# vlongle/pixie

Hardware: AMD Instinct MI355X
Metric: voxels/s (128^3 U-Net fwd) + MPM particle-steps/s (higher is better)
Workload: dtype f32 (operands split fp16 hi+lo, 3 f16 MFMAs/product, fp32 accumulate); 1 GPU; 128^3x64 feature grid -> SegmentationUNet+RegressionUNet forward (+argmax/one-hot combine), 1 scene per GPU per step; grid=128, feature_channels=64, parallelism=scene-parallel x1, executor=c+hip_graph

## Files before the change

include/pixie_hip.h:

```cpp
#ifndef PIXIE_HIP_H
#define PIXIE_HIP_H

#include <stdint.h>

#ifdef __cplusplus
extern "C" {
#endif

const char* pixie_last_error(void);
const char* pixie_build_arch(void);

typedef struct pixie_mpm pixie_mpm;

int pixie_mpm_create(pixie_mpm** out, int n_particles, int n_grid, double grid_lim);
int pixie_mpm_destroy(pixie_mpm* h);
int pixie_mpm_regrid(pixie_mpm* h, int n_grid, double grid_lim, void* stream);

int pixie_mpm_set_field(pixie_mpm* h, const char* name, const void* d_src, int64_t count, void* stream);
int pixie_mpm_get_field(pixie_mpm* h, const char* name, void* d_dst, int64_t count, void* stream);
int pixie_mpm_fill_field(pixie_mpm* h, const char* name, double value, void* stream);

int pixie_mpm_set_scalar(pixie_mpm* h, const char* key, double value);
int pixie_mpm_get_scalar(pixie_mpm* h, const char* key, double* value);

// ... 72 lines not shown
    int32_t in_d, in_h, in_w;
    int32_t upsample;
    int32_t stride;
    int32_t ksize;
    const float* d_pro_a; const float* d_pro_b;
    const float* d_gamma; const float* d_beta;
    int32_t act;
    const float* d_w; const float* d_bias;
    int32_t c_out;
    const float* d_residual;
    float* d_out;
    const void* d_w16;
    const uint32_t* d_in_amax0; const uint32_t* d_in_amax1;
    float in_bound;
    float* d_out_stats;
    uint32_t* d_out_amax;
    void* d_workspace;
    int32_t out_d, out_h, out_w;
    const float* d_skip_in0; int32_t skip_c0;
    const float* d_skip_in1; int32_t skip_c1;
    const void* d_skip_w16; const float* d_skip_bias;
    const uint32_t* d_skip_amax0; const uint32_t* d_skip_amax1;
    int32_t w16_subpixel;
} pixie_conv_desc;

int pixie_conv_cout_padded(int c_out);
int pixie_conv_pack_weights(const float* d_w_oidhw, float* d_w_packed, int c_out, int c_in, int ksize, void* stream);
int64_t pixie_conv_packed16_bytes(int c_out, int c_in, int ksize);
int pixie_conv_pack_weights_f16x2(const float* d_w_oidhw, void* d_packed, int c_out, int c_in, int ksize, void* stream);
int64_t pixie_conv_subpixel_bytes(int c_out, int c_in);
int pixie_conv_pack_weights_subpixel(const float* d_w_oidhw, void* d_packed, int c_out, int c_in, void* stream);
int pixie_conv3d_forward(const pixie_conv_desc* desc, void* stream);
int64_t pixie_conv_stats_floats(const pixie_conv_desc* desc);
int64_t pixie_conv_workspace_bytes(const pixie_conv_desc* desc);
int pixie_stats_finalize(const float* d_stats, const pixie_conv_desc* desc, double* d_sums, void* stream);
int pixie_stats_norm_finalize(const float* d_stats0, const pixie_conv_desc* desc0, double* d_sums0, const float* d_stats1,
                              const pixie_conv_desc* desc1, double* d_sums1, int c1, int64_t spatial, int mode, int groups,
                              double eps, const float* d_weight, const float* d_bias, float* d_a, float* d_b, void* stream);
int pixie_conv_skip_foldable(const pixie_conv_desc* desc);

int pixie_channel_sums(const float* d_x, int channels, int64_t spatial, double* d_sums, void* stream);
int pixie_channel_stats(const float* d_x, int channels, int64_t spatial, double* d_sums, uint32_t* d_amax, void* stream);
int pixie_tensor_amax(const float* d_x, int64_t count, uint32_t* d_slot, void* stream);
int pixie_norm_finalize(const double* d_sums, int channels, int64_t spatial, int mode, int groups, double eps,
                        const float* d_weight, const float* d_bias, float* d_a, float* d_b, void* stream);

// ... 168 lines not shown
```

pixie_amd/_lib.py:

```python
from __future__ import annotations

import ctypes as C
import os

_HERE = os.path.dirname(os.path.abspath(__file__))
LIB_PATH = os.path.join(_HERE, "libpixie_hip.so")
DIAG_LIB_PATH = os.path.join(_HERE, "libpixie_hip_diag.so")


class PixieHipError(RuntimeError):
    pass


class BCDesc(C.Structure):
    _fields_ = [("type", C.c_int32), ("surface_type", C.c_int32), ("reset", C.c_int32), ("pad_", C.c_int32),
                ("point", C.c_double * 3), ("size", C.c_double * 3), ("velocity", C.c_double * 3),
                ("normal", C.c_double * 3), ("start_time", C.c_double), ("end_time", C.c_double),
                ("friction", C.c_double)]


class PModDesc(C.Structure):
    _fields_ = [("type", C.c_int32), ("pad_", C.c_int32),
                ("point", C.c_double * 3), ("size", C.c_double * 3), ("force", C.c_double * 3),
                ("velocity", C.c_double * 3), ("normal", C.c_double * 3), ("h1", C.c_double * 3),
# ... 2 lines not shown
                ("start_time", C.c_double), ("end_time", C.c_double)]


class ConvDesc(C.Structure):
    _fields_ = [("d_in0", C.c_void_p), ("c0", C.c_int32),
                ("d_in1", C.c_void_p), ("c1", C.c_int32),
                ("in_d", C.c_int32), ("in_h", C.c_int32), ("in_w", C.c_int32),
                ("upsample", C.c_int32), ("stride", C.c_int32), ("ksize", C.c_int32),
                ("d_pro_a", C.c_void_p), ("d_pro_b", C.c_void_p),
                ("d_gamma", C.c_void_p), ("d_beta", C.c_void_p),
                ("act", C.c_int32),
                ("d_w", C.c_void_p), ("d_bias", C.c_void_p),
                ("c_out", C.c_int32),
                ("d_residual", C.c_void_p), ("d_out", C.c_void_p),
                ("d_w16", C.c_void_p), ("d_in_amax0", C.c_void_p), ("d_in_amax1", C.c_void_p),
                ("in_bound", C.c_float),
                ("d_out_stats", C.c_void_p), ("d_out_amax", C.c_void_p),
                ("d_workspace", C.c_void_p),
                ("out_d", C.c_int32), ("out_h", C.c_int32), ("out_w", C.c_int32),
                ("d_skip_in0", C.c_void_p), ("skip_c0", C.c_int32),
                ("d_skip_in1", C.c_void_p), ("skip_c1", C.c_int32),
                ("d_skip_w16", C.c_void_p), ("d_skip_bias", C.c_void_p),
                ("d_skip_amax0", C.c_void_p), ("d_skip_amax1", C.c_void_p),
                ("w16_subpixel", C.c_int32)]


class UNetConfigC(C.Structure):
    _fields_ = [("feature_channels", C.c_int32), ("cond_dim", C.c_int32), ("model_channels", C.c_int32), ("num_res_blocks", C.c_int32),
                ("n_channel_mult", C.c_int32), ("channel_mult", C.c_int32 * 8),
                ("n_attention_resolutions", C.c_int32), ("attention_resolutions", C.c_int32 * 8),
                ("grid_size", C.c_int32), ("out_channels", C.c_int32), ("precision", C.c_int32)]


class BatchSched(C.Structure):
    _fields_ = [("dt", C.c_double), ("steps_per_chunk", C.c_int32), ("n_chunks", C.c_int32), ("n_out", C.c_int32), ("pad_", C.c_int32),
                ("shift", C.c_double * 3), ("scale", C.c_double), ("mean", C.c_double * 3), ("inv_rotation", C.c_double * 9),
                ("d_pos", C.c_void_p), ("d_cov", C.c_void_p)]


class BatchSplatOut(C.Structure):
    _fields_ = [("d_log_scale", C.c_void_p), ("d_quat", C.c_void_p)]


class FieldDesc(C.Structure):
    _fields_ = [("d_pred", C.c_void_p), ("d_mask", C.c_void_p),
                ("d_axis_x", C.c_void_p), ("d_axis_y", C.c_void_p), ("d_axis_z", C.c_void_p),
                ("n_classes", C.c_int32), ("d", C.c_int32), ("h", C.c_int32), ("w", C.c_int32),
# ... 170 lines not shown
```

pixie_amd/csrc/conv3d_f16x3.hip:

```cpp
#include <hip/hip_runtime.h>

#include <cstdlib>
#include <map>
#include <string>
#include <type_traits>

#include "../../include/pixie_hip.h"
#include "common.h"
#include "conv_plan.h"

namespace pixie {

typedef float f32x16 __attribute__((ext_vector_type(16)));
typedef _Float16 f16x8 __attribute__((ext_vector_type(8)));

constexpr int kW16HeaderU4 = 4;

struct Conv16Args {
    const float* in0; const float* in1;
    int c0, cin;
    int ID, IH, IW;
    int LD, LH, LW;
    int ups;
    int stride;
// ... 583 lines not shown

__device__ inline void block_channel_sums(const StatParts& P, int c, double* r, double& o1, double& o2) {
    double s1 = 0.0, s2 = 0.0;
    for (int t = threadIdx.x; t < P.n; t += 256) {
        const size_t k = ((size_t)c * P.cstride + (size_t)t * P.tstride) * 2;
        if (P.f64) { const double2 v = *reinterpret_cast<const double2*>(static_cast<const double*>(P.p) + k); s1 += v.x; s2 += v.y; }
        else { const float2 v = *reinterpret_cast<const float2*>(static_cast<const float*>(P.p) + k); s1 += v.x; s2 += v.y; }
    }
    for (int off = 32; off > 0; off >>= 1) { s1 += __shfl_down(s1, off, 64); s2 += __shfl_down(s2, off, 64); }
    if ((threadIdx.x & 63) == 0) { r[2 * (threadIdx.x >> 6)] = s1; r[2 * (threadIdx.x >> 6) + 1] = s2; }
    __syncthreads();
    o1 = r[0] + r[2] + r[4] + r[6]; o2 = r[1] + r[3] + r[5] + r[7];
    __syncthreads();
}

__global__ __launch_bounds__(256) void stats_finalize_kernel(StatParts P, double* __restrict__ sums) {
    const int c = blockIdx.x;
    __shared__ double r[8];
    double s1, s2;
    block_channel_sums(P, c, r, s1, s2);
    if (threadIdx.x == 0) { sums[2 * c] = s1; sums[2 * c + 1] = s2; }
}

__global__ __launch_bounds__(256) void stats_norm_finalize_kernel(StatParts P0, double* sums0, int c0, StatParts P1, double* sums1, int channels,
                                                                  double spatial, int mode, int groups, double eps,
                                                                  const float* __restrict__ weight, const float* __restrict__ bias,
                                                                  float* __restrict__ a, float* __restrict__ b) {
    __shared__ double r[8];
    const int cpg = mode == 0 ? 1 : channels / groups;
    const int first = blockIdx.x * cpg;
    double s1 = 0.0, s2 = 0.0;
    for (int k = first; k < first + cpg; ++k) {
        const bool in0 = k < c0;
        const StatParts& P = in0 ? P0 : P1;
        double* sums = in0 ? sums0 : sums1;
        const int kc = in0 ? k : k - c0;
        double t1, t2;
        if (P.n > 0) {
            block_channel_sums(P, kc, r, t1, t2);
            if (threadIdx.x == 0) { sums[2 * kc] = t1; sums[2 * kc + 1] = t2; }
        } else {
            t1 = sums[2 * kc]; t2 = sums[2 * kc + 1];
        }
        s1 += t1; s2 += t2;
    }
    const double cnt = mode == 0 ? spatial : spatial * cpg;
    const double mean = s1 / cnt;
    double var = s2 / cnt - mean * mean;
    if (var < 0.0) var = 0.0;
    const double rstd = 1.0 / sqrt(var + eps);
    for (int k = first + threadIdx.x; k < first + cpg; k += 256) {
        if (mode == 0) {
            a[k] = (float)rstd;
            b[k] = (float)(-mean * rstd);
        } else {
            const double w = weight ? (double)weight[k] : 1.0;
            const double bb = bias ? (double)bias[k] : 0.0;
            a[k] = (float)(rstd * w);
            b[k] = (float)(bb - mean * rstd * w);
        }
    }
}

__global__ __launch_bounds__(256) void splitk_reduce_kernel(const float* __restrict__ partial, int slices, long n_elems, long osp,
                                                            const float* __restrict__ bias, const float* residual, float* out) {
    const long i = (long)blockIdx.x * 256 + threadIdx.x;
    if (i >= n_elems) return;
    float v = partial[i];
    for (int s = 1; s < slices; ++s) v += partial[(size_t)s * n_elems + i];
    if (bias) v += bias[i / osp];
    if (residual) v += residual[i];
    out[i] = v;
}

constexpr int kReduceSeg = 4096;
template <bool VEC>
__global__ __launch_bounds__(256) void splitk_reduce_stats_kernel(const float* __restrict__ partial, int slices, long n_elems, long osp,
                                                                  const float* __restrict__ bias, const float* residual, float* out,
                                                                  double* __restrict__ stats, unsigned* out_amax) {
    const int c = blockIdx.y;
    const long seg0 = (long)blockIdx.x * kReduceSeg;
    const size_t base = (size_t)c * osp;
    const float bv = bias ? bias[c] : 0.0f;
    double s1 = 0.0, s2 = 0.0;
    float mx = 0.0f;
    if (VEC) {
#pragma unroll
        for (int k = 0; k < kReduceSeg / 1024; ++k) {
            const long j = seg0 + k * 1024 + (long)threadIdx.x * 4;
            if (j < osp) {
                const size_t i = base + j;
                float4 v = *reinterpret_cast<const float4*>(partial + i);
                for (int s = 1; s < slices; ++s) {
                    const float4 q = *reinterpret_cast<const float4*>(partial + (size_t)s * n_elems + i);
                    v.x += q.x; v.y += q.y; v.z += q.z; v.w += q.w;
                }
                if (bias) { v.x += bv; v.y += bv; v.z += bv; v.w += bv; }
                if (residual) {
                    const float4 q = *reinterpret_cast<const float4*>(residual + i);
                    v.x += q.x; v.y += q.y; v.z += q.z; v.w += q.w;
                }
                *reinterpret_cast<float4*>(out + i) = v;
// ... 11 lines not shown
                const size_t i = base + j;
                float v = partial[i];
                for (int s = 1; s < slices; ++s) v += partial[(size_t)s * n_elems + i];
                if (bias) v += bv;
                if (residual) v += residual[i];
                out[i] = v;
                const double x = v;
                s1 += x; s2 += x * x; mx = fmaxf(mx, fabsf(v));
            }
        }
    }
    for (int off = 32; off > 0; off >>= 1) {
        s1 += __shfl_down(s1, off, 64);
        s2 += __shfl_down(s2, off, 64);
        mx = fmaxf(mx, __shfl_down(mx, off, 64));
    }
    __shared__ double r[8];
    __shared__ float rmx[4];
    const int lane = threadIdx.x & 63, wave = threadIdx.x >> 6;
    if (lane == 0) { r[2 * wave] = s1; r[2 * wave + 1] = s2; rmx[wave] = mx; }
    __syncthreads();
    if (threadIdx.x == 0) {
        double* dst = stats + ((size_t)c * gridDim.x + blockIdx.x) * 2;
        dst[0] = r[0] + r[2] + r[4] + r[6];
        dst[1] = r[1] + r[3] + r[5] + r[7];
        const unsigned m = __float_as_uint(fmaxf(fmaxf(rmx[0], rmx[1]), fmaxf(rmx[2], rmx[3])));
        if (out_amax && m > __hip_atomic_load(out_amax, __ATOMIC_RELAXED, __HIP_MEMORY_SCOPE_AGENT)) atomicMax(out_amax, m);
    }
}

__global__ __launch_bounds__(256) void amax_kernel(const float* __restrict__ x, long n, unsigned* __restrict__ slot) {
    float m = 0.0f;
    const long stride = (long)gridDim.x * 256 * 4;
    long i = ((long)blockIdx.x * 256 + threadIdx.x) * 4;
    if ((reinterpret_cast<size_t>(x) & 15) == 0) {
        for (; i + 3 < n; i += stride) {
            const float4 v = *reinterpret_cast<const float4*>(x + i);
            m = fmaxf(fmaxf(m, fabsf(v.x)), fmaxf(fabsf(v.y), fmaxf(fabsf(v.z), fabsf(v.w))));
        }
        for (long k = i; k < n && k < i + 4; ++k) m = fmaxf(m, fabsf(x[k]));
    } else {
        for (long k = (long)blockIdx.x * 256 + threadIdx.x; k < n; k += (long)gridDim.x * 256) m = fmaxf(m, fabsf(x[k]));
    }
    for (int off = 32; off > 0; off >>= 1) m = fmaxf(m, __shfl_down(m, off, 64));
    if ((threadIdx.x & 63) == 0 && m > 0.0f) atomicMax(slot, __float_as_uint(m));
}

__global__ void pack_weights_f16x2_kernel(const float* __restrict__ src, uint4* __restrict__ dst, int cout, int cin, int taps,
                                          int coutp, const unsigned* __restrict__ amax_bits) {
    const int KG = cin >> 3;
// ... 221 lines not shown
int conv3d_f16x3_forward(const pixie_conv_desc* d, const ConvPlan& p, hipStream_t st) {
    PX_REQUIRE(p.refusal != CONV_BAD_STRIDE, "f16x3 conv: stride must be 1, or 2 for a 3^3 kernel");
    PX_REQUIRE(p.refusal != CONV_BAD_CHANNELS, "f16x3 conv: c_in must be a multiple of 16 (got %d+%d)", d->c0, d->c1);
    PX_REQUIRE(d->d_in_amax0 != nullptr || d->in_bound > 0.0f, "f16x3 conv: needs d_in_amax0 or a positive in_bound");
    PX_REQUIRE(d->c1 == 0 || d->d_in_amax0 == nullptr || d->d_in_amax1 != nullptr, "f16x3 conv: second input needs its own amax slot");
    PX_REQUIRE(p.refusal != CONV_BAD_SUBPIXEL, "f16x3 conv: sub-pixel weights need upsample = 1, ksize = 3, stride = 1 and no folded skip");
    Conv16Args a = conv16_args(d, p);
    a.w16 = reinterpret_cast<const uint4*>(d->d_w16);
    a.amax0 = d->d_in_amax0; a.amax1 = (d->c1 > 0) ? d->d_in_amax1 : nullptr; a.in_bound = d->in_bound;
    a.stats = d->d_out_stats; a.out_amax = d->d_out_amax;
    if (d->d_skip_w16) {
        PX_REQUIRE(p.skip_foldable, "f16x3 conv: this launch cannot fold a skip convolution (pixie_conv_skip_foldable)");
        PX_REQUIRE(d->d_skip_in0 && d->d_skip_amax0 && (d->skip_c1 == 0 || (d->d_skip_in1 && d->d_skip_amax1)), "f16x3 conv: folded skip needs its inputs and their amax slots");
        a.sk_in0 = d->d_skip_in0; a.sk_in1 = d->d_skip_in1; a.sk_c0 = d->skip_c0; a.sk_cin = d->skip_c0 + d->skip_c1;
        a.sk_w16 = reinterpret_cast<const uint4*>(d->d_skip_w16); a.sk_bias = d->d_skip_bias;
        a.sk_amax0 = d->d_skip_amax0; a.sk_amax1 = d->skip_c1 > 0 ? d->d_skip_amax1 : nullptr;
    }
    if (p.slices > 1) {
        a.partial = static_cast<float*>(d->d_workspace);
        a.stats = nullptr; a.out_amax = nullptr;
    }
    PX_REQUIRE(p.refusal != CONV_BAD_LDS, "f16x3 conv: tile needs %zu B of LDS", p.lds_bytes);
    PX_REQUIRE(p.f16x3(), "f16x3 conv: bad sizes");
    if (int rc = launch(conv16_kernel(p), p, a, st)) return rc;
    if (p.slices == 1) return 0;
    const long osp = (long)a.OD * a.OH * a.OW, n_elems = (long)a.cout * osp;
    if (d->d_out_stats) {
        const dim3 rgrid((unsigned)reduce_segments(osp), (unsigned)a.cout);
        double* rstats = reinterpret_cast<double*>(d->d_out_stats);
        PX_REQUIRE((reinterpret_cast<size_t>(rstats) & 7) == 0, "f16x3 conv: d_out_stats of a split-K launch must be 8-byte aligned");
        const bool vec = osp % 4 == 0 && ((reinterpret_cast<size_t>(a.partial) | reinterpret_cast<size_t>(a.residual) | reinterpret_cast<size_t>(a.out)) & 15) == 0;
        if (vec) hipLaunchKernelGGL(splitk_reduce_stats_kernel<true>, rgrid, dim3(256), 0, st, a.partial, p.slices, n_elems, osp, a.bias, a.residual,
                                    a.out, rstats, d->d_out_amax);
        else hipLaunchKernelGGL(splitk_reduce_stats_kernel<false>, rgrid, dim3(256), 0, st, a.partial, p.slices, n_elems, osp, a.bias, a.residual,
                                a.out, rstats, d->d_out_amax);
    } else {
        hipLaunchKernelGGL(splitk_reduce_kernel, dim3((unsigned)((n_elems + 255) / 256)), dim3(256), 0, st, a.partial, p.slices, n_elems, osp,
                           a.bias, a.residual, a.out);
    }
    PX_CHECK_HIP(hipGetLastError());
    return 0;
}

int conv3d_exact_forward(const pixie_conv_desc* d, const ConvPlan& p, hipStream_t st) {
    PX_REQUIRE(p.refusal != CONV_BAD_LDS, "exact conv: tile needs %zu B of LDS", p.lds_bytes);
    PX_REQUIRE(p.path == CONV_EXACT_TILED, "exact conv: bad sizes");
    Conv16Args a = conv16_args(d, p);
    a.wf = d->d_w;
    a.in_bound = 1.0f;
    return launch(conv16_kernel(p), p, a, st);
}

}

using namespace pixie;

static ConvPlan plan_of(const pixie_conv_desc* d) { return d ? conv_plan(conv_shape_of(d)) : ConvPlan{}; }
static StatParts stat_parts(const ConvPlan& p, const void* stats) { return StatParts{stats, p.stats.n, p.stats.cstride, p.stats.tstride, p.stats.f64}; }
// ... 116 lines not shown
```

pixie_amd/csrc/conv3d_mfma.hip:

```cpp
#include <hip/hip_runtime.h>

#include "../../include/pixie_hip.h"
#include "common.h"
#include "conv_plan.h"

namespace pixie {

typedef float f32x16 __attribute__((ext_vector_type(16)));

struct ConvArgs {
    const float* in0; const float* in1;
    int c0, cin;
    int ID, IH, IW;
    int LD, LH, LW;
    int ups;
    int stride;
    int OD, OH, OW;
    const float* pro_a; const float* pro_b; const float* gamma; const float* beta;
    int act;
    const float* w; const float* bias;
    int cout, coutp;
    const float* residual; float* out;
    int TX, TY, TZ, lTX, lTY;
    int tiles_x, tiles_y, tiles_z;
// ... 177 lines not shown
    const int taps = ksize * ksize * ksize;
    const int coutp = pixie_conv_cout_padded(c_out);
    const long total = (long)taps * c_in * coutp;
    hipLaunchKernelGGL(pack_weights_kernel, dim3(cdiv(total, 256)), dim3(256), 0, as_stream(stream), d_w, d_packed, c_out, c_in, taps, coutp);
    PX_CHECK_HIP(hipGetLastError());
    return 0;
}

extern "C" int pixie_conv3d_forward(const pixie_conv_desc* d, void* stream) {
    PX_REQUIRE(d && d->d_in0 && (d->d_w || d->d_w16) && d->d_out, "pixie_conv3d_forward: null pointer in descriptor");
    PX_REQUIRE(d->ksize == 1 || d->ksize == 3, "pixie_conv3d_forward: ksize must be 1 or 3 (got %d)", d->ksize);
    PX_REQUIRE(d->stride == 1 || d->stride == 2, "pixie_conv3d_forward: stride must be 1 or 2 (got %d)", d->stride);
    PX_REQUIRE(d->upsample == 0 || d->upsample == 1, "pixie_conv3d_forward: upsample must be 0 or 1");
    PX_REQUIRE(d->c0 > 0 && d->c1 >= 0 && (d->c1 == 0 || d->d_in1), "pixie_conv3d_forward: bad channel split");
    PX_REQUIRE(d->c_out > 0 && d->in_d > 0 && d->in_h > 0 && d->in_w > 0, "pixie_conv3d_forward: bad sizes");
    PX_REQUIRE((d->d_pro_a == nullptr) == (d->d_pro_b == nullptr), "pixie_conv3d_forward: pro_a/pro_b must come together");
    PX_REQUIRE((d->d_gamma == nullptr) == (d->d_beta == nullptr), "pixie_conv3d_forward: gamma/beta must come together");
    PX_REQUIRE(!(d->d_gamma && d->upsample) || (d->d_w16 && d->w16_subpixel),
               "pixie_conv3d_forward: spatial affine with upsample needs the sub-pixel path (w16_subpixel), with gamma/beta of the stored grid");

    const ConvPlan p = conv_plan(conv_shape_of(d));
    if (d->d_w16) return conv3d_f16x3_forward(d, p, as_stream(stream));
    PX_REQUIRE(!d->d_skip_w16, "pixie_conv3d_forward: a folded skip convolution needs the f16x3 path (d_w16)");
    if (p.path != CONV_FIRST_GEN) return conv3d_exact_forward(d, p, as_stream(stream));

    ConvArgs a{};
    a.in0 = d->d_in0; a.in1 = d->d_in1; a.c0 = d->c0; a.cin = d->c0 + d->c1;
    a.ID = d->in_d; a.IH = d->in_h; a.IW = d->in_w;
    a.ups = p.ups; a.LD = p.LD; a.LH = p.LH; a.LW = p.LW;
    a.stride = d->stride;
    a.OD = p.OD; a.OH = p.OH; a.OW = p.OW;
    a.pro_a = d->d_pro_a; a.pro_b = d->d_pro_b; a.gamma = d->d_gamma; a.beta = d->d_beta; a.act = d->act;
    a.w = d->d_w; a.bias = d->d_bias; a.cout = d->c_out; a.coutp = pixie_conv_cout_padded(d->c_out);
    a.residual = d->d_residual; a.out = d->d_out;

    const long ovol = (long)a.OD * a.OH * a.OW;
    int MB = (a.coutp >= 64) ? 2 : 1;
    int NB = 4;
    auto n_wg = [&](int mb, int nb) {
        const long tiles = (ovol + 128L * nb - 1) / (128L * nb);
        return tiles * ((a.coutp + mb * 32 - 1) / (mb * 32));
    };
    while (n_wg(MB, NB) < 512 && NB > 1) NB /= 2;
    if (n_wg(MB, NB) < 512 && MB > 1) MB = 1;
    if (a.stride == 2 && NB > 2) NB = 2;

// ... 24 lines not shown
```

pixie_amd/csrc/unet_exec.hip:

```cpp
#include <hip/hip_runtime.h>

#include <algorithm>
#include <cmath>
#include <cstdlib>
#include <cstring>
#include <map>
#include <memory>
#include <stdexcept>
#include <string>
#include <tuple>
#include <unordered_map>
#include <vector>

#include "../../include/pixie_hip.h"
#include "common.h"
#include "conv_plan.h"

namespace pixie {
int channel_stats_prezeroed(const float* d_x, int channels, int64_t spatial, double* d_sums, uint32_t* d_amax, hipStream_t st);
int norm_finalize_cat(const double* d_sums0, int c0, const double* d_sums1, int c1, int64_t spatial, int mode, int groups, double eps,
                      const float* d_weight, const float* d_bias, float* d_a, float* d_b, hipStream_t st);
namespace {

enum { ACT_NONE = 0, ACT_LEAKY = 1, ACT_SILU = 2 };
// ... 172 lines not shown
        used_.erase(u);
        auto next = free_.lower_bound(off);
        if (next != free_.end() && off + size == next->first) { size += next->second; next = free_.erase(next); }
        if (next != free_.begin()) {
            auto prev = std::prev(next);
            if (prev->first + prev->second == off) { prev->second += size; return; }
        }
        free_[off] = size;
    }
    template <class T> T* ptr(int64_t off) const { return reinterpret_cast<T*>(base + off); }
};

struct Exec;
struct Tens {
    Exec* ex = nullptr;
    float* p = nullptr;
    int64_t off = -1;
    int c = 0, d = 0, h = 0, w = 0;
    int64_t sums_off = -1;
    bool has_sums = false;
    double* sums = nullptr;
    int64_t partials_off = -1;
    pixie_conv_desc pdesc;
    uint32_t* slot = nullptr;
    int64_t spatial() const { return (int64_t)d * h * w; }
    ~Tens();
};
using TP = std::shared_ptr<Tens>;

struct Packed { void* d = nullptr; uint64_t version = ~0ull; };
struct Sized { int64_t bytes; int slots; int64_t zsum_doubles; };
struct Bound { float wmax = 0, bmax = 0; uint64_t wver = ~0ull, bver = ~0ull; };

}
}

using namespace pixie;

struct pixie_unet {
    Cfg cfg;
    Plan plan;
    std::vector<Param> params;
    std::unordered_map<std::string, int> index;
    std::unordered_map<std::string, Packed> packed32, packed16;
    std::unordered_map<std::string, Bound> bounds;
    uint32_t* d_bound_slots = nullptr;
    std::vector<uint32_t> h_bound_slots;
    std::map<std::tuple<int, int, int, bool>, Sized> sized;
    bool fuse_stats = true, split_k = true, fold_skip = true, subpixel = true;
    bool split_stats = true;
    struct Replay { const float* feat; const float* proj0; float* out; void* ws; int d; uint64_t epoch; hipGraph_t graph; hipGraphExec_t exec; };
    bool use_graph = false;
    uint64_t epoch = 0;
    std::vector<Replay> replays;
    static constexpr size_t kMaxReplays = 4;
    void drop_replay(size_t i) {
        (void)hipGraphExecDestroy(replays[i].exec);
        (void)hipGraphDestroy(replays[i].graph);
        replays.erase(replays.begin() + (long)i);
    }

    const Param& param(const std::string& key) const {
        auto it = index.find(key);
        if (it == index.end()) fail("pixie_unet: no parameter named '%s'", key.c_str());
        return params[it->second];
    }
};

namespace pixie {
namespace {

struct Exec {
    pixie_unet* net = nullptr;
    Arena arena;
    bool dry = false;
    void* stream = nullptr;
    uint32_t* slots = nullptr;
    int slot_next = 0, slot_cap = 0;
    double* zsums = nullptr;
    int64_t zsum_next = 0, zsum_cap = 0;

    TP make(int c, int d, int h, int w) {
        auto t = std::make_shared<Tens>();
        t->ex = this; t->c = c; t->d = d; t->h = h; t->w = w;
        t->off = arena.alloc((int64_t)c * d * h * w * sizeof(float));
        t->p = arena.ptr<float>(t->off);
        return t;
    }
    TP external(const float* p, int c, int d, int h, int w) {
        auto t = std::make_shared<Tens>();
        t->ex = this; t->p = const_cast<float*>(p); t->c = c; t->d = d; t->h = h; t->w = w;
        return t;
    }
    uint32_t* new_slot() {
        if (!dry && slot_next >= slot_cap) fail("pixie_unet_forward: out of |x|max slots (internal sizing error)");
        return dry ? (slot_next++, nullptr) : slots + slot_next++;
    }
    struct Scratch {
        Exec* ex; int64_t off;
        Scratch(Exec* e, int64_t bytes) : ex(e), off(e->arena.alloc(bytes)) {}
        ~Scratch() { ex->arena.release(off); }
        template <class T> T* as() const { return ex->arena.ptr<T>(off); }
    };

    const float* P(const std::string& key) {
        const Param& p = net->param(key);
        if (!dry && !p.d) fail("pixie_unet_forward: parameter '%s' was never set", key.c_str());
        return p.d;
    }
    const void* w16(const std::string& key, bool subpixel = false) {
        const Param& p = net->param(key + ".weight");
        if (dry) return nullptr;
        Packed& e = net->packed16[subpixel ? key + "#subpixel" : key];
        if (e.version != p.version) {
            const int cout = (int)p.shape[0], cin = (int)p.shape[1], k = (int)p.shape[2];
            const int64_t nb = subpixel ? (k == 3 ? pixie_conv_subpixel_bytes(cout, cin) : 0) : pixie_conv_packed16_bytes(cout, cin, k);
            if (nb <= 0) fail("pixie_unet: '%s' cannot take the f16x3 packing (c_in %d)", key.c_str(), cin);
            if (!e.d && hipMalloc(&e.d, (size_t)nb) != hipSuccess) fail("pixie_unet: hipMalloc of %lld bytes failed", (long long)nb);
            if (!p.d) fail("pixie_unet_forward: parameter '%s.weight' was never set", key.c_str());
// ... 14 lines not shown
            const int64_t nb = taps * cin * pixie_conv_cout_padded(cout) * (int64_t)sizeof(float);
            if (!e.d && hipMalloc(&e.d, (size_t)nb) != hipSuccess) fail("pixie_unet: hipMalloc of %lld bytes failed", (long long)nb);
            if (!p.d) fail("pixie_unet_forward: parameter '%s.weight' was never set", key.c_str());
            ok(pixie_conv_pack_weights(p.d, static_cast<float*>(e.d), cout, cin, k, stream), "pixie_conv_pack_weights");
            e.version = p.version;
        }
        return static_cast<const float*>(e.d);
    }
    float norm_bound(const std::string& key, int64_t count) {
        if (dry) return 1.0f;
        const Bound& b = net->bounds[key];
        return (float)(std::sqrt((double)count) * (double)b.wmax + (double)b.bmax + 1e-30);
    }

    void stats(const TP& t) {
        if (t->has_sums || t->partials_off >= 0) return;
        t->has_sums = true;
        if (!dry && zsum_next + 2 * t->c > zsum_cap) fail("pixie_unet_forward: out of statistics space (internal sizing error)");
        t->sums = dry ? nullptr : zsums + zsum_next;
        zsum_next += 2 * t->c;
        t->slot = new_slot();
        if (!dry) ok(channel_stats_prezeroed(t->p, t->c, t->spatial(), t->sums, t->slot, as_stream(stream)), "pixie_channel_stats");
    }
    struct AB { std::shared_ptr<Scratch> mem; float* a; float* b; };
    AB norm_finalize(const std::vector<TP>& parts, int64_t spatial, int mode, int groups, const float* w, const float* b) {
        for (auto& t : parts) stats(t);
        const Tens* t0 = parts[0].get();
        const Tens* t1 = parts.size() > 1 ? parts[1].get() : nullptr;
        const int c0 = t0->c, c1 = t1 ? t1->c : 0, c = c0 + c1;
        AB r;
        const int cpad = (c + 63) / 64 * 64;
        r.mem = std::make_shared<Scratch>(this, (int64_t)(cpad + c) * sizeof(float));
        r.a = r.mem->as<float>();
        r.b = r.a + cpad;
        const bool p0 = t0->partials_off >= 0, p1 = t1 && t1->partials_off >= 0;
        if (p0 || p1) {
            pixie_conv_desc d0 = t0->pdesc;
            if (!p0) { std::memset(&d0, 0, sizeof d0); d0.c_out = c0; }
            if (!dry) ok(pixie_stats_norm_finalize(p0 ? arena.ptr<float>(t0->partials_off) : nullptr, &d0, t0->sums,
                                                   p1 ? arena.ptr<float>(t1->partials_off) : nullptr, p1 ? &t1->pdesc : nullptr, t1 ? t1->sums : nullptr,
                                                   c1, spatial, mode, groups, 1e-5, w, b, r.a, r.b, stream), "pixie_stats_norm_finalize");
            for (auto& t : parts)
                if (t->partials_off >= 0) { arena.release(t->partials_off); t->partials_off = -1; t->has_sums = true; }
        } else if (!t1) {
            if (!dry) ok(pixie_norm_finalize(t0->sums, c, spatial, mode, groups, 1e-5, w, b, r.a, r.b, stream), "pixie_norm_finalize");
        } else {
            if (!dry) ok(norm_finalize_cat(t0->sums, c0, t1->sums, c1, spatial, mode, groups, 1e-5, w, b, r.a, r.b, as_stream(stream)), "pixie_norm_finalize");
        }
// ... 56 lines not shown
        if (!f16) {
            desc.d_w = w32(wkey);
            if (!dry) ok(pixie_conv3d_forward(&desc, stream), "pixie_conv3d_forward");
            return out;
        }
        desc.d_w16 = w16(wkey, s.subpixel);
        desc.w16_subpixel = s.subpixel ? 1 : 0;
        if (o.skip_parts) {
            const std::vector<TP>& sp = *o.skip_parts;
            desc.d_skip_in0 = sp[0]->p; desc.skip_c0 = sp[0]->c;
            desc.d_skip_in1 = sp.size() > 1 ? sp[1]->p : nullptr; desc.skip_c1 = sp.size() > 1 ? sp[1]->c : 0;
            desc.d_skip_w16 = w16(o.skip_key);
            desc.d_skip_bias = P(o.skip_key + ".bias");
            desc.d_skip_amax0 = sp[0]->slot; desc.d_skip_amax1 = sp.size() > 1 ? sp[1]->slot : nullptr;
        }
        if (raw) {
            desc.d_in_amax0 = parts[0]->slot;
            desc.d_in_amax1 = x1 ? parts[1]->slot : nullptr;
        } else {
            desc.in_bound = o.bound;
        }
        std::unique_ptr<Scratch> workspace;
        if (plan.workspace_bytes > 0) { workspace.reset(new Scratch(this, plan.workspace_bytes)); desc.d_workspace = workspace->as<void>(); }
        bool have_stats = false;
        if (net->fuse_stats) {
            uint32_t* slot = new_slot();
            const int64_t nfl = plan.stats_floats;
            if (nfl > 0 && (!workspace || net->split_stats)) {
                out->partials_off = arena.alloc(nfl * (int64_t)sizeof(float));
                desc.d_out_stats = arena.ptr<float>(out->partials_off);
                desc.d_out_amax = slot;
                have_stats = true;
                out->slot = slot;
            }
        }
        if (!dry) ok(pixie_conv3d_forward(&desc, stream), "pixie_conv3d_forward");
        if (have_stats) {
            out->sums_off = arena.alloc((int64_t)cout * 2 * sizeof(double));
            out->sums = arena.ptr<double>(out->sums_off);
            out->pdesc = desc;
        }
        return out;
    }

    TP res(const Blk& b, const std::vector<TP>& parts) {
        const std::string& p = b.prefix;
        const int64_t spatial = parts[0]->spatial();
        AB pro = norm_finalize(parts, spatial, 0, 1, nullptr, nullptr);
        ConvOpt o1; o1.pro = &pro; o1.affine_store = p + ".in_layers.0"; o1.act = ACT_LEAKY; o1.bound = norm_bound(p + ".in_layers.0", spatial);
        TP h = conv(parts, p + ".in_layers.2", b.cout, 3, o1);
        AB pro2 = norm_finalize({h}, spatial, 0, 1, nullptr, nullptr);
        TP skip = parts[0];
        ConvOpt o2; o2.pro = &pro2; o2.affine_store = p + ".out_layers.0"; o2.act = ACT_LEAKY; o2.bound = norm_bound(p + ".out_layers.0", spatial);
        if (b.cin != b.cout) {
            if (net->fold_skip && skip_foldable(h, b.cout, 3, parts)) {
                skip.reset();
                for (auto& t : parts) stats(t);
                o2.skip_parts = &parts; o2.skip_key = p + ".skip_connection";
            } else {
                skip = conv(parts, p + ".skip_connection", b.cout, 1, ConvOpt{});
            }
        }
        o2.residual = skip;
// ... 73 lines not shown
            TP skip = hs.back(); hs.pop_back();
            if (skip->d != h->d || skip->h != h->h || skip->w != h->w) fail("pixie_unet_forward: skip tensor and decoder tensor differ in size");
            std::vector<TP> parts{h, skip};
            h.reset(); skip.reset();
            for (const Blk& b : seq) {
                TP nh = block(b, parts, (b.kind == UP && !hs.empty()) ? hs.back().get() : nullptr);
                parts.clear();
                parts.push_back(nh);
            }
            h = parts[0];
        }
        AB pro = norm_finalize({h}, h->spatial(), 0, 1, nullptr, nullptr);
        ConvOpt oo; oo.pro = &pro; oo.affine_store = "unet.out.0"; oo.act = ACT_LEAKY; oo.bound = norm_bound("unet.out.0", h->spatial());
        oo.out_ptr = d_out;
        return conv({h}, "unet.out.2", c.out_channels, 3, oo);
    }
};

Tens::~Tens() {
    if (!ex) return;
    if (off >= 0) ex->arena.release(off);
    if (sums_off >= 0) ex->arena.release(sums_off);
    if (partials_off >= 0) ex->arena.release(partials_off);
}

void refresh_bounds(pixie_unet* net, void* stream) {
    std::vector<std::pair<std::string, int>> todo;
    int n_norm = 0;
    for (const Param& p : net->params) {
        if (!p.norm || p.key.size() < 7 || p.key.compare(p.key.size() - 7, 7, ".weight") != 0) continue;
        const std::string key = p.key.substr(0, p.key.size() - 7);
        const Param& pb = net->param(key + ".bias");
        Bound& b = net->bounds[key];
        if (b.wver != p.version || b.bver != pb.version) todo.push_back({key, 2 * n_norm});
        ++n_norm;
    }
    if (todo.empty()) return;
    const size_t bytes = (size_t)2 * n_norm * sizeof(uint32_t);
    if (!net->d_bound_slots && hipMalloc(&net->d_bound_slots, bytes) != hipSuccess) fail("pixie_unet: hipMalloc failed");
    net->h_bound_slots.assign((size_t)2 * n_norm, 0u);
    hipStream_t s = as_stream(stream);
    if (hipMemsetAsync(net->d_bound_slots, 0, bytes, s) != hipSuccess) fail("pixie_unet: hipMemsetAsync failed");
    for (auto& t : todo) {
        const Param& pw = net->param(t.first + ".weight");
        const Param& pb = net->param(t.first + ".bias");
        if (!pw.d || !pb.d) fail("pixie_unet_forward: parameter '%s' was never set", t.first.c_str());
// ... 47 lines not shown

extern "C" int pixie_unet_create(pixie_unet** out, const pixie_unet_config* c) {
    PX_REQUIRE(out && c, "pixie_unet_create: null argument");
    PX_REQUIRE(c->n_channel_mult >= 1 && c->n_channel_mult <= 8 && c->n_attention_resolutions >= 0 && c->n_attention_resolutions <= 8,
               "pixie_unet_create: channel_mult needs 1..8 entries, attention_resolutions 0..8");
    PX_REQUIRE(c->feature_channels > 0 && c->cond_dim > 0 && c->model_channels > 0 && c->num_res_blocks > 0 && c->grid_size > 0 && c->out_channels > 0,
               "pixie_unet_create: non-positive size");
    PX_REQUIRE(c->precision == 0 || c->precision == 1, "pixie_unet_create: precision is 0 (f16x3) or 1 (exact fp32)");
    return guarded([&] {
        std::unique_ptr<pixie_unet> n(new pixie_unet);
        n->cfg.feature_channels = c->feature_channels; n->cfg.cond_dim = c->cond_dim; n->cfg.model_channels = c->model_channels;
        n->cfg.num_res_blocks = c->num_res_blocks; n->cfg.grid_size = c->grid_size; n->cfg.out_channels = c->out_channels;
        n->cfg.precision = c->precision;
        n->cfg.mult.assign(c->channel_mult, c->channel_mult + c->n_channel_mult);
        n->cfg.attn.assign(c->attention_resolutions, c->attention_resolutions + c->n_attention_resolutions);
        n->plan = build_plan(n->cfg);
        n->params = param_table(n->cfg, n->plan);
        for (size_t i = 0; i < n->params.size(); ++i) n->index[n->params[i].key] = (int)i;
        const char* fs = getenv("PIXIE_FUSE_STATS"); n->fuse_stats = !(fs && fs[0] == '0');
        const char* sk = getenv("PIXIE_CONV_SPLIT_K"); n->split_k = !(sk && sk[0] == '0');
        const char* fk = getenv("PIXIE_FOLD_SKIP"); n->fold_skip = !(fk && fk[0] == '0');
        const char* ss = getenv("PIXIE_SPLIT_STATS"); n->split_stats = !(ss && ss[0] == '0');
        const char* sx = getenv("PIXIE_CONV_SUBPIXEL"); n->subpixel = !(sx && sx[0] == '0');
        *out = n.release();
        return 0;
    });
}

extern "C" int pixie_unet_destroy(pixie_unet* h) {
    if (!h) return 0;
    for (auto& kv : h->packed16) if (kv.second.d) (void)hipFree(kv.second.d);
    for (auto& kv : h->packed32) if (kv.second.d) (void)hipFree(kv.second.d);
    if (h->d_bound_slots) (void)hipFree(h->d_bound_slots);
    while (!h->replays.empty()) h->drop_replay(0);
    delete h;
    return 0;
}

extern "C" int pixie_unet_param_count(const pixie_unet* h) { return h ? (int)h->params.size() : 0; }

extern "C" int pixie_unet_param_info(const pixie_unet* h, int i, const char** key, int64_t* numel, int32_t* ndim, int64_t shape[5]) {
    PX_REQUIRE(h && i >= 0 && i < (int)h->params.size(), "pixie_unet_param_info: index out of range");
    const Param& p = h->params[i];
    if (key) *key = p.key.c_str();
    if (numel) *numel = p.numel;
    if (ndim) *ndim = (int32_t)p.shape.size();
// ... 94 lines not shown
```

pixie_amd/unet.py:

```python
from __future__ import annotations

import ctypes as C
import math
import os
import warnings
import weakref
from typing import Dict, List, Optional, Sequence, Tuple

import torch
import torch.nn as nn

from . import _lib
from ._lib import ConvDesc, check
from .unet_plan import Block, UNetConfig, UNetPlan, build_plan, param_shapes, is_norm_key

ACT_NONE, ACT_LEAKY, ACT_SILU = 0, 1, 2
DEFAULT_PRECISION = os.environ.get("PIXIE_CONV_PRECISION", "f16x3")
_ZERO_INIT_SUFFIXES = (".out_layers.3.weight", ".out_layers.3.bias", ".proj_out.weight", ".proj_out.bias",
                       "unet.out.2.weight", "unet.out.2.bias")


def _ptr(t: Optional[torch.Tensor]):
    return C.c_void_p(t.data_ptr()) if t is not None else C.c_void_p(0)

# ... 49 lines not shown
        desc.d_skip_w16 = addr(skip["w16"])
        desc.d_skip_bias = addr(skip["bias"])
        desc.d_skip_amax0 = addr(skip["amax"][0])
        desc.d_skip_amax1 = addr(skip["amax"][1]) if len(sp) > 1 else None
    stats = workspace = None
    if w16 is not None and split_k:
        wsb = lib.pixie_conv_workspace_bytes(C.byref(desc))
        if wsb > 0:
            workspace = alloc((wsb,), torch.uint8)
            desc.d_workspace = addr(workspace)
    if out_amax is not None and w16 is not None:
        nfl = lib.pixie_conv_stats_floats(C.byref(desc))
        if nfl > 0 and (workspace is None or split_stats):
            stats = alloc((nfl,), torch.float32)
            desc.d_out_stats = addr(stats)
            desc.d_out_amax = addr(out_amax)
    return desc, out, stats, workspace


class PendingStats:

    def __init__(self, stats: torch.Tensor, desc: ConvDesc, cout: int):
        self.stats, self.desc, self.cout = stats, desc, cout


class HipOps:

    def __init__(self, device: torch.device):
        if device.type != "cuda":
            raise _lib.PixieHipError("pixie_amd U-Net operators run on a HIP device only (no CPU fallback)")
        self.device = device
        self.lib = _lib.load()
        self.split_k = os.environ.get("PIXIE_CONV_SPLIT_K", "1") != "0"
        self.record_variant = False
        self.last_variant = (0, 1)

    @property
    def stream(self):
        return _lib.current_stream_ptr()

    def pack_conv(self, weight: torch.Tensor) -> torch.Tensor:
        cout, cin = weight.shape[0], weight.shape[1]
        k = weight.shape[2]
        coutp = self.lib.pixie_conv_cout_padded(cout)
        w = weight.detach().to(self.device, torch.float32).contiguous()
        taps = 1
# ... 33 lines not shown
             affine: Optional[Tuple[torch.Tensor, torch.Tensor]] = None, act: int = ACT_NONE,
             residual: Optional[torch.Tensor] = None, w16: Optional[torch.Tensor] = None,
             in_amax: Optional[Sequence[torch.Tensor]] = None, in_bound: float = 0.0,
             out_amax: Optional[torch.Tensor] = None, out_size: Optional[Tuple[int, int, int]] = None,
             skip: Optional[dict] = None, subpixel: bool = False, defer_stats: bool = False, split_stats: bool = True):
        desc, out, stats, _ = fill_conv_desc(
            self.lib, lambda shape, dtype: torch.empty(shape, device=self.device, dtype=dtype), parts, packed_w, bias, cout, ksize,
            stride=stride, upsample=upsample, pro=pro, affine=affine, act=act, residual=residual, w16=w16, in_amax=in_amax,
            in_bound=in_bound, out_amax=out_amax, out_size=out_size, skip=skip, subpixel=subpixel, split_k=self.split_k,
            split_stats=defer_stats and split_stats)
        sums = None
        if self.record_variant:
            sl = C.c_int(1)
            self.last_variant = (int(_lib.load(diag=True).pixie_conv_kernel_variant(C.byref(desc), C.byref(sl))), int(sl.value))
        check(self.lib.pixie_conv3d_forward(C.byref(desc), self.stream), "pixie_conv3d_forward")
        if desc.d_out_stats:
            if defer_stats:
                sums = PendingStats(stats, desc, cout)
            else:
                sums = self.stats_finalize(PendingStats(stats, desc, cout))
        if out_amax is not None:
            return out, sums
        return out

    def skip_foldable(self, x: torch.Tensor, cout: int, ksize: int, skip_parts: Sequence[torch.Tensor]) -> bool:
        desc = ConvDesc()
        desc.c0 = x.shape[0]
        desc.in_d, desc.in_h, desc.in_w = (int(v) for v in x.shape[1:])
        desc.stride, desc.ksize, desc.c_out = 1, ksize, cout
        desc.d_w16 = 1
        desc.d_workspace = 1 if self.split_k else None
        desc.skip_c0 = skip_parts[0].shape[0]
        desc.skip_c1 = skip_parts[1].shape[0] if len(skip_parts) > 1 else 0
        return bool(self.lib.pixie_conv_skip_foldable(C.byref(desc)))

    def channel_sums(self, x: torch.Tensor) -> torch.Tensor:
        c = x.shape[0]
        spatial = x.numel() // c
        sums = torch.empty((c, 2), device=self.device, dtype=torch.float64)
        check(self.lib.pixie_channel_sums(_ptr(x), c, spatial, _ptr(sums), self.stream), "pixie_channel_sums")
        return sums

    def channel_stats(self, x: torch.Tensor, amax_slot: torch.Tensor) -> torch.Tensor:
        c = x.shape[0]
        spatial = x.numel() // c
        sums = torch.empty((c, 2), device=self.device, dtype=torch.float64)
# ... 603 lines not shown
```

Before: 24.50 million voxels/s.

## Finalise per-channel norm stats inside split-K reduce via last-block counter

The split-K reduce kernel now finishes the norm statistics itself. Each block publishes its partial sums, bumps a per-channel atomic counter, and the last block to arrive reduces all segments, then writes the sums and the per-channel scale/shift (rstd, -mean*rstd). This removes the separate stats/norm finalize launch and its partial-buffer traffic for mode-0 single-input norms in the U-Net executor. The cost is extra atomics, fences and a tail reduction by one block per channel, plus per-channel counter slots that must be reset to zero for graph replay.

```diff
diff --git a/include/pixie_hip.h b/include/pixie_hip.h
--- a/include/pixie_hip.h
+++ b/include/pixie_hip.h
@@ -118,6 +118,10 @@
     const void* d_skip_w16; const float* d_skip_bias;
     const uint32_t* d_skip_amax0; const uint32_t* d_skip_amax1;
     int32_t w16_subpixel;
+    uint32_t* d_fin_counters;
+    double* d_fin_sums;
+    float* d_fin_a; float* d_fin_b;
+    double fin_eps;
 } pixie_conv_desc;
 
 int pixie_conv_cout_padded(int c_out);
diff --git a/pixie_amd/_lib.py b/pixie_amd/_lib.py
--- a/pixie_amd/_lib.py
+++ b/pixie_amd/_lib.py
@@ -48,7 +48,9 @@
                 ("d_skip_in1", C.c_void_p), ("skip_c1", C.c_int32),
                 ("d_skip_w16", C.c_void_p), ("d_skip_bias", C.c_void_p),
                 ("d_skip_amax0", C.c_void_p), ("d_skip_amax1", C.c_void_p),
-                ("w16_subpixel", C.c_int32)]
+                ("w16_subpixel", C.c_int32),
+                ("d_fin_counters", C.c_void_p), ("d_fin_sums", C.c_void_p), ("d_fin_a", C.c_void_p), ("d_fin_b", C.c_void_p),
+                ("fin_eps", C.c_double)]
 
 
 class UNetConfigC(C.Structure):
diff --git a/pixie_amd/csrc/conv3d_f16x3.hip b/pixie_amd/csrc/conv3d_f16x3.hip
--- a/pixie_amd/csrc/conv3d_f16x3.hip
+++ b/pixie_amd/csrc/conv3d_f16x3.hip
@@ -629,6 +629,13 @@
     if (threadIdx.x == 0) { sums[2 * c] = s1; sums[2 * c + 1] = s2; }
 }
 
+__device__ __forceinline__ void mean_rstd(double s1, double s2, double cnt, double eps, double& mean, double& rstd) {
+    mean = s1 / cnt;
+    double var = s2 / cnt - mean * mean;
+    if (var < 0.0) var = 0.0;
+    rstd = 1.0 / sqrt(var + eps);
+}
+
 __global__ __launch_bounds__(256) void stats_norm_finalize_kernel(StatParts P0, double* sums0, int c0, StatParts P1, double* sums1, int channels,
                                                                   double spatial, int mode, int groups, double eps,
                                                                   const float* __restrict__ weight, const float* __restrict__ bias,
@@ -652,10 +659,8 @@
         s1 += t1; s2 += t2;
     }
     const double cnt = mode == 0 ? spatial : spatial * cpg;
-    const double mean = s1 / cnt;
-    double var = s2 / cnt - mean * mean;
-    if (var < 0.0) var = 0.0;
-    const double rstd = 1.0 / sqrt(var + eps);
+    double mean, rstd;
+    mean_rstd(s1, s2, cnt, eps, mean, rstd);
     for (int k = first + threadIdx.x; k < first + cpg; k += 256) {
         if (mode == 0) {
             a[k] = (float)rstd;
@@ -680,11 +685,12 @@
     out[i] = v;
 }
 
+struct ReduceFinalise { unsigned* counters; double* sums; float* a; float* b; double spatial, eps; };
 constexpr int kReduceSeg = 4096;
 template <bool VEC>
 __global__ __launch_bounds__(256) void splitk_reduce_stats_kernel(const float* __restrict__ partial, int slices, long n_elems, long osp,
                                                                   const float* __restrict__ bias, const float* residual, float* out,
-                                                                  double* __restrict__ stats, unsigned* out_amax) {
+                                                                  double* __restrict__ stats, unsigned* out_amax, ReduceFinalise F) {
     const int c = blockIdx.y;
     const long seg0 = (long)blockIdx.x * kReduceSeg;
     const size_t base = (size_t)c * osp;
@@ -742,10 +748,46 @@
     __syncthreads();
     if (threadIdx.x == 0) {
         double* dst = stats + ((size_t)c * gridDim.x + blockIdx.x) * 2;
-        dst[0] = r[0] + r[2] + r[4] + r[6];
-        dst[1] = r[1] + r[3] + r[5] + r[7];
+        const double v1 = r[0] + r[2] + r[4] + r[6], v2 = r[1] + r[3] + r[5] + r[7];
+        if (F.a && gridDim.x > 1) {
+            __hip_atomic_store(reinterpret_cast<unsigned long long*>(dst), (unsigned long long)__double_as_longlong(v1), __ATOMIC_RELAXED, __HIP_MEMORY_SCOPE_AGENT);
+            __hip_atomic_store(reinterpret_cast<unsigned long long*>(dst) + 1, (unsigned long long)__double_as_longlong(v2), __ATOMIC_RELAXED, __HIP_MEMORY_SCOPE_AGENT);
+        } else {
+            dst[0] = v1; dst[1] = v2;
+        }
         const unsigned m = __float_as_uint(fmaxf(fmaxf(rmx[0], rmx[1]), fmaxf(rmx[2], rmx[3])));
         if (out_amax && m > __hip_atomic_load(out_amax, __ATOMIC_RELAXED, __HIP_MEMORY_SCOPE_AGENT)) atomicMax(out_amax, m);
+    }
+    if (!F.a) return;
+    const int nseg = (int)gridDim.x;
+    if (nseg > 1) {
+        __shared__ int last;
+        if (threadIdx.x == 0) {
+            asm volatile("s_waitcnt vmcnt(0) lgkmcnt(0)" ::: "memory");
+            const unsigned prev = __hip_atomic_fetch_add(F.counters + c, 1u, __ATOMIC_RELAXED, __HIP_MEMORY_SCOPE_AGENT);
+            last = prev == (unsigned)(nseg - 1);
+            if (last) {
+                __builtin_amdgcn_fence(__ATOMIC_ACQUIRE, "agent");
+                asm volatile("s_waitcnt vmcnt(0)" ::: "memory");
+            }
+        }
+        __syncthreads();
+        if (!last) return;
+    } else {
+        __syncthreads();
+    }
+    const StatParts P{stats, nseg, (long)nseg, 1L, 1};
+    double t1, t2;
+    block_channel_sums(P, c, r, t1, t2);
+    if (threadIdx.x == 0) {
+        F.sums[2 * c] = t1; F.sums[2 * c + 1] = t2;
+        double q1 = 0.0, q2 = 0.0;
+        q1 += t1; q2 += t2;
+        double mean, rstd;
+        mean_rstd(q1, q2, F.spatial, F.eps, mean, rstd);
+        F.a[c] = (float)rstd;
+        F.b[c] = (float)(-mean * rstd);
+        if (nseg > 1) __hip_atomic_store(F.counters + c, 0u, __ATOMIC_RELAXED, __HIP_MEMORY_SCOPE_AGENT);
     }
 }
 
@@ -1013,6 +1055,11 @@
     }
     PX_REQUIRE(p.refusal != CONV_BAD_LDS, "f16x3 conv: tile needs %zu B of LDS", p.lds_bytes);
     PX_REQUIRE(p.f16x3(), "f16x3 conv: bad sizes");
+    if (d->d_fin_a) {
+        PX_REQUIRE(p.slices > 1 && d->d_out_stats, "f16x3 conv: d_fin_a needs a split-K launch that takes d_out_stats (pixie_conv_workspace_bytes > 0): "
+                   "only its reduce finalises in-launch");
+        PX_REQUIRE(d->d_fin_counters && d->d_fin_sums && d->d_fin_b && d->fin_eps > 0.0, "f16x3 conv: d_fin_a needs d_fin_counters, d_fin_sums, d_fin_b and a positive fin_eps");
+    }
     if (int rc = launch(conv16_kernel(p), p, a, st)) return rc;
     if (p.slices == 1) return 0;
     const long osp = (long)a.OD * a.OH * a.OW, n_elems = (long)a.cout * osp;
@@ -1021,10 +1068,11 @@
         double* rstats = reinterpret_cast<double*>(d->d_out_stats);
         PX_REQUIRE((reinterpret_cast<size_t>(rstats) & 7) == 0, "f16x3 conv: d_out_stats of a split-K launch must be 8-byte aligned");
         const bool vec = osp % 4 == 0 && ((reinterpret_cast<size_t>(a.partial) | reinterpret_cast<size_t>(a.residual) | reinterpret_cast<size_t>(a.out)) & 15) == 0;
+        const ReduceFinalise fin{d->d_fin_counters, d->d_fin_sums, d->d_fin_a, d->d_fin_b, (double)osp, d->fin_eps};
         if (vec) hipLaunchKernelGGL(splitk_reduce_stats_kernel<true>, rgrid, dim3(256), 0, st, a.partial, p.slices, n_elems, osp, a.bias, a.residual,
-                                    a.out, rstats, d->d_out_amax);
+                                    a.out, rstats, d->d_out_amax, fin);
         else hipLaunchKernelGGL(splitk_reduce_stats_kernel<false>, rgrid, dim3(256), 0, st, a.partial, p.slices, n_elems, osp, a.bias, a.residual,
-                                a.out, rstats, d->d_out_amax);
+                                a.out, rstats, d->d_out_amax, fin);
     } else {
         hipLaunchKernelGGL(splitk_reduce_kernel, dim3((unsigned)((n_elems + 255) / 256)), dim3(256), 0, st, a.partial, p.slices, n_elems, osp,
                            a.bias, a.residual, a.out);
diff --git a/pixie_amd/csrc/conv3d_mfma.hip b/pixie_amd/csrc/conv3d_mfma.hip
--- a/pixie_amd/csrc/conv3d_mfma.hip
+++ b/pixie_amd/csrc/conv3d_mfma.hip
@@ -223,6 +223,7 @@
     const ConvPlan p = conv_plan(conv_shape_of(d));
     if (d->d_w16) return conv3d_f16x3_forward(d, p, as_stream(stream));
     PX_REQUIRE(!d->d_skip_w16, "pixie_conv3d_forward: a folded skip convolution needs the f16x3 path (d_w16)");
+    PX_REQUIRE(!d->d_fin_a, "pixie_conv3d_forward: the in-launch finalise (d_fin_a) needs the f16x3 path (d_w16)");
     if (p.path != CONV_FIRST_GEN) return conv3d_exact_forward(d, p, as_stream(stream));
 
     ConvArgs a{};
diff --git a/pixie_amd/csrc/unet_exec.hip b/pixie_amd/csrc/unet_exec.hip
--- a/pixie_amd/csrc/unet_exec.hip
+++ b/pixie_amd/csrc/unet_exec.hip
@@ -218,6 +218,8 @@
     double* sums = nullptr;
     int64_t partials_off = -1;
     pixie_conv_desc pdesc;
+    int64_t ab_off = -1;
+    float* fa = nullptr; float* fb = nullptr;
     uint32_t* slot = nullptr;
     int64_t spatial() const { return (int64_t)d * h * w; }
     ~Tens();
@@ -245,6 +247,7 @@
     std::map<std::tuple<int, int, int, bool>, Sized> sized;
     bool fuse_stats = true, split_k = true, fold_skip = true, subpixel = true;
     bool split_stats = true;
+    bool inlaunch_fin = true;
     struct Replay { const float* feat; const float* proj0; float* out; void* ws; int d; uint64_t epoch; hipGraph_t graph; hipGraphExec_t exec; };
     bool use_graph = false;
     uint64_t epoch = 0;
@@ -291,6 +294,12 @@
     uint32_t* new_slot() {
         if (!dry && slot_next >= slot_cap) fail("pixie_unet_forward: out of |x|max slots (internal sizing error)");
         return dry ? (slot_next++, nullptr) : slots + slot_next++;
+    }
+    uint32_t* new_slots(int n) {
+        if (!dry && slot_next + n > slot_cap) fail("pixie_unet_forward: out of |x|max slots (internal sizing error)");
+        uint32_t* p = dry ? nullptr : slots + slot_next;
+        slot_next += n;
+        return p;
     }
     struct Scratch {
         Exec* ex; int64_t off;
@@ -351,8 +360,9 @@
         t->slot = new_slot();
         if (!dry) ok(channel_stats_prezeroed(t->p, t->c, t->spatial(), t->sums, t->slot, as_stream(stream)), "pixie_channel_stats");
     }
-    struct AB { std::shared_ptr<Scratch> mem; float* a; float* b; };
+    struct AB { std::shared_ptr<Scratch> mem; float* a; float* b; TP owner; };
     AB norm_finalize(const std::vector<TP>& parts, int64_t spatial, int mode, int groups, const float* w, const float* b) {
+        if (mode == 0 && parts.size() == 1 && parts[0]->fa) return AB{nullptr, parts[0]->fa, parts[0]->fb, parts[0]};
         for (auto& t : parts) stats(t);
         const Tens* t0 = parts[0].get();
         const Tens* t1 = parts.size() > 1 ? parts[1].get() : nullptr;
@@ -455,7 +465,7 @@
         }
         std::unique_ptr<Scratch> workspace;
         if (plan.workspace_bytes > 0) { workspace.reset(new Scratch(this, plan.workspace_bytes)); desc.d_workspace = workspace->as<void>(); }
-        bool have_stats = false;
+        bool have_stats = false, fin = false;
         if (net->fuse_stats) {
             uint32_t* slot = new_slot();
             const int64_t nfl = plan.stats_floats;
@@ -465,13 +475,27 @@
                 desc.d_out_amax = slot;
                 have_stats = true;
                 out->slot = slot;
+                fin = net->inlaunch_fin && plan.stats.f64;
             }
         }
-        if (!dry) ok(pixie_conv3d_forward(&desc, stream), "pixie_conv3d_forward");
         if (have_stats) {
             out->sums_off = arena.alloc((int64_t)cout * 2 * sizeof(double));
             out->sums = arena.ptr<double>(out->sums_off);
-            out->pdesc = desc;
+        }
+        if (fin) {
+            const int cpad = (cout + 63) / 64 * 64;
+            out->ab_off = arena.alloc((int64_t)(cpad + cout) * sizeof(float));
+            out->fa = arena.ptr<float>(out->ab_off);
+            out->fb = out->fa + cpad;
+            desc.d_fin_counters = new_slots(cout);
+            desc.d_fin_sums = out->sums; desc.d_fin_a = out->fa; desc.d_fin_b = out->fb; desc.fin_eps = 1e-5;
+        }
+        if (!dry) ok(pixie_conv3d_forward(&desc, stream), "pixie_conv3d_forward");
+        if (have_stats) out->pdesc = desc;
+        if (fin) {
+            arena.release(out->partials_off);
+            out->partials_off = -1;
+            out->has_sums = true;
         }
         return out;
     }
@@ -591,6 +615,7 @@
     if (off >= 0) ex->arena.release(off);
     if (sums_off >= 0) ex->arena.release(sums_off);
     if (partials_off >= 0) ex->arena.release(partials_off);
+    if (ab_off >= 0) ex->arena.release(ab_off);
 }
 
 void refresh_bounds(pixie_unet* net, void* stream) {
@@ -684,6 +709,7 @@
         const char* fk = getenv("PIXIE_FOLD_SKIP"); n->fold_skip = !(fk && fk[0] == '0');
         const char* ss = getenv("PIXIE_SPLIT_STATS"); n->split_stats = !(ss && ss[0] == '0');
         const char* sx = getenv("PIXIE_CONV_SUBPIXEL"); n->subpixel = !(sx && sx[0] == '0');
+        const char* fi = getenv("PIXIE_INLAUNCH_FINALISE"); n->inlaunch_fin = !(fi && fi[0] == '0');
         *out = n.release();
         return 0;
     });
diff --git a/pixie_amd/unet.py b/pixie_amd/unet.py
--- a/pixie_amd/unet.py
+++ b/pixie_amd/unet.py
@@ -95,6 +95,7 @@
 
     def __init__(self, stats: torch.Tensor, desc: ConvDesc, cout: int):
         self.stats, self.desc, self.cout = stats, desc, cout
+        self.sums = self.a = self.b = None
 
 
 class HipOps:
@@ -174,6 +175,20 @@
         if out_amax is not None:
             return out, sums
         return out
+
+    def conv_finalised(self, parts: Sequence[torch.Tensor], bias: Optional[torch.Tensor], cout: int, ksize: int, out_amax: torch.Tensor,
+                       fin_counters: torch.Tensor, fin_eps: float = 1e-5, **kw):
+        desc, out, stats, _ = fill_conv_desc(
+            self.lib, lambda shape, dtype: torch.empty(shape, device=self.device, dtype=dtype), parts, None, bias, cout, ksize,
+            out_amax=out_amax, split_k=self.split_k, split_stats=True, **kw)
+        pend = PendingStats(stats, desc, cout)
+        pend.sums = torch.empty((cout, 2), device=self.device, dtype=torch.float64)
+        pend.a = torch.empty(cout, device=self.device, dtype=torch.float32)
+        pend.b = torch.empty(cout, device=self.device, dtype=torch.float32)
+        desc.d_fin_counters, desc.d_fin_sums, desc.d_fin_a, desc.d_fin_b = _ptr(fin_counters), _ptr(pend.sums), _ptr(pend.a), _ptr(pend.b)
+        desc.fin_eps = fin_eps
+        check(self.lib.pixie_conv3d_forward(C.byref(desc), self.stream), "pixie_conv3d_forward")
+        return out, pend
 
     def skip_foldable(self, x: torch.Tensor, cout: int, ksize: int, skip_parts: Sequence[torch.Tensor]) -> bool:
         desc = ConvDesc()
```

After: 24.47 million voxels/s. No clear change (-0.1%).
